# Tzq2doc/distributed_learning_simulator

Measured on AMD Instinct MI355X. Metric: FL rounds/sec (FedAvg, 100 clients, ResNet-18, CIFAR-10-shaped), higher is better.
Workload: dtype fp32; 1 GPU; fedavg_resnet18; model=ResNet18, algo=fed_avg, clients=100, local_epochs=5, global_batch=6400, per_client_batch=64, parallelism=client-dp1, backend=hip

## Files before the change

### csrc/bindings.cpp

```cpp
#include <pybind11/pybind11.h>

#include <algorithm>
#include <optional>
#include <stdexcept>
#include <string>
#include <vector>

#include "dls.h"

namespace py = pybind11;
typedef uintptr_t ptr;

template <typename T>
static T* P(ptr p) {
  return reinterpret_cast<T*>(p);
}
static hipStream_t S(ptr s) { return reinterpret_cast<hipStream_t>(s); }

extern "C" const char* dls_src_hash();

class Args {
 public:
  struct Ptr {
    uintptr_t v;
// ... 255 lines not shown
    p.coef = a.p("coef", 0); p.relu = a.i("relu", 0); p.x_valid = a.p("x_valid", 0);
    p.valid_img = a.p("valid_img", 0); p.dw = a.p("dw"); p.dw_cs = a.l("dw_cs"); p.part = a.p("part", 0);
    p.K = a.i("K"); p.B = a.i("B"); p.H = a.i("H"); p.W = a.i("W"); p.C = a.i("C"); p.N = a.i("N");
    const int xm = a.i("xm"), dm = a.i("dm");
    const hipStream_t s = a.p("s");
    a.finish();
    return halo_wgrad(p, xm, dm, s);
  });
  m.def("conv_halo_bn_dense_supported", &conv_halo_bn_dense_supported);
  m.def("conv_halo_bn_dense_fwd", [](py::kwargs kw) {
    Args a(kw, "conv_halo_bn_dense_fwd");
    const auto x = a.p("x"), coef = a.p("coef"), valid_rows = a.p("valid_rows", 0), wsplit = a.p("wsplit");
    const auto y = a.p("y"), stats = a.p("stats", 0), stats_valid = a.p("stats_valid", 0), s = a.p("s");
    const auto ny = a.p("ny", 0), mask = a.p("mask", 0);
    const long x_cs = a.l("x_cs"), ws_cs = a.l("ws_cs"), ws_plane = a.l("ws_plane"), y_cs = a.l("y_cs");
    const long ny_cs = a.l("ny_cs", 0);
    const int ldx = a.i("ldx"), creal = a.i("creal"), relu = a.i("relu", 0), rep = a.i("rep"), ldy = a.i("ldy");
    const int K = a.i("K"), B = a.i("B"), H = a.i("H"), W = a.i("W"), C = a.i("C"), N = a.i("N"), ldny = a.i("ldny", 0);
    a.finish();
    return conv_halo_bn_dense_fwd(x, x_cs, ldx, creal, coef, relu, valid_rows, wsplit, ws_cs, ws_plane, rep, y, y_cs,
                                  ldy, K, B, H, W, C, N, stats, stats_valid, ny, ny_cs, ldny, mask, s);
  });
  m.def("bn_bwd", [](py::kwargs kw) {
    Args a(kw, "bn_bwd");
    const auto dy = a.p("dy"), x = a.p("x"), y = a.p("y", 0), mean = a.p("mean", 0);
    const auto rstd = a.p("rstd", 0), gamma = a.p("gamma", 0), valid_rows = a.p("valid_rows", 0);
    const auto dx = a.p("dx", 0), dpre = a.p("dpre", 0), dgamma = a.p("dgamma", 0);
    const auto dbeta = a.p("dbeta", 0), ws = a.p("ws"), relu_mask = a.p("relu_mask", 0), s = a.p("s");
    const auto dxp = a.p("dxp", 0), pre_part = a.p("pre_part", 0), coef_ext = a.p("coef_ext", 0);
    const long g_cs = a.l("g_cs", 0), dg_cs = a.l("dg_cs", 0);
    const int K = a.i("K"), R = a.i("R"), C = a.i("C"), relu = a.i("relu", 0), f32 = a.i("f32");
    const int ldx = a.i("ldx", 0), acc_dx = a.i("acc_dx", 0), dx_f32 = a.i("dx_f32", 1);
    const int pre_nparts = a.i("pre_nparts", 0), stage = a.i("stage", 0);
    a.finish();
    bn_bwd(dy, x, y, mean, rstd, gamma, valid_rows, g_cs, K, R, C, relu, dx, dpre, dgamma, dbeta, dg_cs, ws, relu_mask,
           f32, s, ldx, acc_dx, dxp, dx_f32, pre_part, pre_nparts, coef_ext, stage);
  });
  m.def("ln_fwd", [](ptr x, ptr gamma, ptr beta, ptr y, ptr mean, ptr rstd, long g_cs, int K, long rpc, int C,
                     float eps, int rep, int f32, ptr s, ptr yp) {
    ln_fwd(P<const void>(x), P<const void>(gamma), P<const void>(beta), P<void>(y), P<float>(mean), P<float>(rstd),
           g_cs, K, rpc, C, eps, rep, f32, S(s), P<bf16_t>(yp));
  });
  m.def("ln_bwd", [](ptr dy, ptr x, ptr mean, ptr rstd, ptr gamma, long g_cs, int K, long rpc, int C, ptr dx,
                     ptr dgamma, ptr dbeta, long dg_cs, int f32, ptr s, ptr ws) {
    ln_bwd(P<const void>(dy), P<const void>(x), P<const float>(mean), P<const float>(rstd), P<const void>(gamma), g_cs,
           K, rpc, C, P<void>(dx), P<float>(dgamma), P<float>(dbeta), dg_cs, P<float>(ws), f32, S(s));
  });
  m.def("ln_workspace_floats", &ln_workspace_floats);
  m.def("gn_shape_ok", &gn_shape_ok);
  m.def("gn_workspace_floats", &gn_workspace_floats);
  m.def("gn_fwd", [](ptr x, ptr res, ptr gamma, ptr beta, ptr y, ptr yp, ptr mean, ptr rstd, ptr valid, long g_cs,
                     int rep, int K, int B, int HW, int C, int G, float eps, int relu, int f32, ptr s) {
    gn_fwd(P<const void>(x), P<const void>(res), P<const void>(gamma), P<const void>(beta), P<void>(y), P<bf16_t>(yp),
           P<float>(mean), P<float>(rstd), P<const int>(valid), g_cs, rep, K, B, HW, C, G, eps, relu, f32, S(s));
  });
  m.def("gn_bwd", [](ptr dy, ptr x, ptr y, ptr mean, ptr rstd, ptr gamma, ptr valid, long g_cs, int rep, int K, int B,
                     int HW, int C, int G, int relu, ptr dx, ptr dres, ptr dgamma, ptr dbeta, long dg_cs, ptr ws,
                     int f32, ptr s) {
    gn_bwd(P<const void>(dy), P<const void>(x), P<const void>(y), P<const float>(mean), P<const float>(rstd),
           P<const void>(gamma), P<const int>(valid), g_cs, rep, K, B, HW, C, G, relu, P<void>(dx), P<void>(dres),
           P<float>(dgamma), P<float>(dbeta), dg_cs, P<float>(ws), f32, S(s));
  });
  m.def("col_sum_workspace_floats", &col_sum_workspace_floats);
  m.def("col_sum", [](ptr x, ptr out, long out_cs, int K, long rows, int C, int f32, ptr s, ptr ws) {
    col_sum(P<const void>(x), P<float>(out), out_cs, K, rows, C, f32, S(s), P<float>(ws));
  });

  m.def("pool_fwd", [](ptr x, ptr y, ptr idx, int K, int B, int H, int W, int C, int OH, int OW, int k, int stride,
                       int pad, int mode, int f32, ptr s) {
// ... 248 lines not shown
```

### csrc/dls.h

```cpp
#pragma once
#include <hip/hip_runtime.h>
#include <stdint.h>

typedef uint16_t bf16_t;

constexpr int kOptUnset = -1000000;
extern int g_opt_attn_mfma, g_opt_conv_gl, g_opt_pl_min_wg;
extern int g_opt_halo_wgrad_unroll;
extern int g_opt_halo_skip;
extern int g_opt_conv_pix;
int native_option(int& slot, const char* env, int dflt);
bool set_native_option(const char* name, int value);

struct FastDiv {
  uint32_t d, mul, shift;
};

static inline FastDiv make_fastdiv(uint32_t d) {
  FastDiv f;
  f.d = d;
  uint32_t s = 0;
  while ((1u << s) < d) ++s;
  f.shift = s;
  f.mul = (uint32_t)((((uint64_t)1 << 32) * (((uint64_t)1 << s) - d)) / d + 1);
// ... 255 lines not shown
                 int ldy_x = 0, const int* valid_rows = nullptr);
void conv_halo_set_mode(int m);
void conv_halo_set_variant(int v);
bool conv_tn_pl_supported(const ConvTNParams& p);
bool conv_tn_pl(ConvTNParams p, int K, int variant, hipStream_t s);
int conv_tn_pl_num_variants();
int conv_tn_pl_variant();
void conv_tn_pl_set_variant(int v);
int conv_tn_pl_splitk(int K, int Co, int R, int M, int variant);
void tn_fold(const float* part, float* dw, long dw_cs, int K, int splitk, long CoR, hipStream_t s,
             const SgdEpi* sgd = nullptr);
int conv_tn_f32_num_variants();
int conv_tn_f32_splitk(int K, int Co, int R, int M, int gco, int gc, int variant);
bool conv_tn_f32_bn_bwd_ok(int K, int Co, int R, int gco, int gc, int variant);

long bn_workspace_floats(int K, long R, int C);
void bn_fwd(const void* x, const void* gamma, const void* beta, const void* res, void* y, float* mean, float* rstd,
            const int* valid_rows, long g_cs, int K, int R, int C, int relu, float eps, int rep, float* ws,
            uint8_t* relu_mask, int f32, hipStream_t s,
            int ldx = 0, const float* pre_part = nullptr,
            int pre_nparts = 0, bf16_t* yp = nullptr,
            int y_f32 = 1, float* coef_out = nullptr, int apply = 1,
            const float* res_coef = nullptr,
            int res_relu = 0);
void bn_bwd(const void* dy, const void* x, const void* y, const float* mean, const float* rstd, const void* gamma,
            const int* valid_rows, long g_cs, int K, int R, int C, int relu, void* dx, void* dpre, float* dgamma,
            float* dbeta, long dg_cs, float* ws, const uint8_t* relu_mask, int f32,
            hipStream_t s, int ldx = 0,
            int acc_dx = 0, bf16_t* dxp = nullptr,
            int dx_f32 = 1,
            const float* pre_part = nullptr,
            int pre_nparts = 0,
            float* coef_ext = nullptr,
            int stage = 0);
void ln_fwd(const void* x, const void* gamma, const void* beta, void* y, float* mean, float* rstd, long g_cs, int K,
            long rows_per_client, int C, float eps, int rep, int f32, hipStream_t s,
            bf16_t* yp = nullptr);
void ln_bwd(const void* dy, const void* x, const float* mean, const float* rstd, const void* gamma, long g_cs, int K,
            long rows_per_client, int C, void* dx, float* dgamma, float* dbeta, long dg_cs, float* ws, int f32,
            hipStream_t s);
long col_sum_workspace_floats(int K, long rows, int C);
long ln_workspace_floats(int K, long rows_per_client, int C);
bool gn_shape_ok(int HW, int C, int G);
long gn_workspace_floats(int K, int B, int C);
void gn_fwd(const void* x, const void* res, const void* gamma, const void* beta, void* y, bf16_t* yp, float* mean,
            float* rstd, const int* valid, long g_cs, int rep, int K, int B, int HW, int C, int G, float eps, int relu,
            int f32, hipStream_t s);
void gn_bwd(const void* dy, const void* x, const void* y, const float* mean, const float* rstd, const void* gamma,
            const int* valid, long g_cs, int rep, int K, int B, int HW, int C, int G, int relu, void* dx, void* dres,
            float* dgamma, float* dbeta, long dg_cs, float* ws, int f32, hipStream_t s);
void col_sum(const void* x, float* out, long out_cs, int K, long rows, int C, int f32, hipStream_t s,
             float* ws = nullptr);

void pool_fwd(const void* x, void* y, int* idx, int K, int B, int H, int W, int C, int OH, int OW, int k, int stride,
              int pad, int mode, int f32, hipStream_t s);
void pool_bwd(const void* dy, const int* idx, void* dx, int K, int B, int H, int W, int C, int OH, int OW, int k,
              int stride, int pad, int mode, int f32, hipStream_t s);
void gap_fwd(const void* x, void* y, int KB, int HW, int C, int f32, hipStream_t s);
void gap_bwd(const void* dy, void* dx, int KB, int HW, int C, int f32, hipStream_t s);
void ce_fwd_bwd(const void* logits, const int* labels, const int* valid, float* loss, float* correct, void* dlogits,
                int K, int B, int NC, int f32, hipStream_t s, float* rowbuf = nullptr);
void relu_bwd(const void* dy, const void* y, void* dx, long n, int f32, hipStream_t s);

void quant_pack(const float* x, long ld, const int* seg, const int64_t* seg_off, const int64_t* seg_numel,
                const uint8_t* bits, const float* lo, const float* scale, const int64_t* seg_byte_off,
                const int64_t* row_off, int K, int nseg, long P, int stochastic, const uint32_t* seeds, uint8_t* out,
                hipStream_t s);
// ... 140 lines not shown
```

### csrc/norm.hip

```cpp
#include "common.h"
#include <algorithm>
#include <numeric>

#include "dls.h"

namespace {

constexpr int ROWS_PER_BLOCK = 512;

static int rows_per_block(long R, int K) {
  const long want = std::min<long>(64, (2048 + K - 1) / K);
  const long bpc = std::max(1L, std::min(want, std::max(1L, R / 64)));
  return (int)std::min<long>(ROWS_PER_BLOCK, (R + bpc - 1) / bpc);
}

struct BNCoefArgs {
  const void* gamma;
  const void* beta;
  const float* mean_in;
  const float* rstd_in;
  float* mean_out;
  float* rstd_out;
  float* coef;
  float* dgamma;
  float* dbeta;
  long dg_cs, g_cs;
  float eps;
  int rep, bwd;
};

template <typename T>
__device__ __forceinline__ void bn_coef_math(float s0, float s1, int k, int c, int C, float n, const BNCoefArgs& a) {
  const long i = (long)k * C + c;
  const float g = ldf(static_cast<const T*>(a.gamma) + (long)(k / a.rep) * a.g_cs + c);
  if (!a.bwd) {
// ... 349 lines not shown
#pragma unroll
            for (int j = 0; j < V; ++j) out[j] += fmaxf(fmaf(rv[j], rsc[j], rsh[j]), 0.f);
          } else if (res_coef) {
#pragma unroll
            for (int j = 0; j < V; ++j) out[j] += fmaf(rv[j], rsc[j], rsh[j]);
          } else {
#pragma unroll
            for (int j = 0; j < V; ++j) out[j] += rv[j];
          }
        }
        if (relu) {
#pragma unroll
          for (int j = 0; j < V; ++j) out[j] = fmaxf(out[j], 0.f);
        }
      } else {
#pragma unroll
        for (int j = 0; j < V; ++j) out[j] = 0.f;
      }
      if (rmask) {
        uint32_t m = 0;
#pragma unroll
        for (int j = 0; j < V; ++j) m |= (rt<T>(out[j]) > 0.f ? 1u : 0u) << j;
        rmask[((long)k * R + r) * (C / 8) + c0 / 8] = (uint8_t)m;
      }
      if (y_f32) store_vec<V>(y + off, out);
      if (yp) {
        bf16_t* hp = yp + (long)k * R * C + off;
        store_planes<V>(hp, hp + (long)R * C, out);
      }
    }
  }
}

template <typename T, int V>
__global__ void __launch_bounds__(256) bn_bwd_apply_kernel(const T* __restrict__ dy, const T* __restrict__ x,
                                                           const T* __restrict__ y,
                                                           const int* __restrict__ valid_rows,
                                                           const float* __restrict__ coef, int R, int C, int relu,
                                                           T* __restrict__ dx, T* __restrict__ dpre,
                                                           int rpb, const uint8_t* __restrict__ rmask, int ldx,
                                                           int acc_dx, bf16_t* __restrict__ dxp, int dx_f32) {
  const int k = blockIdx.y;
  const int CT = C / V;
  const int nvalid = valid_rows ? min(valid_rows[k], R) : R;
  const int r0 = blockIdx.x * rpb, r1 = min(R, r0 + rpb);
  const long base = (long)k * R * C, base_x = (long)k * R * ldx;
  for (int cg = 0; cg < CT; cg += 256) {
    const int ctn = min(256, CT - cg);
    const int RT = 256 / ctn;
    const int cc = threadIdx.x % ctn, rl = threadIdx.x / ctn;
    if (rl >= RT) continue;
    const int c0 = (cg + cc) * V;
    float ca[V], cd[V], ce[V];
#pragma unroll
    for (int j = 0; j < V; ++j) {
      const long q = 3 * ((long)k * C + c0 + j);
      ca[j] = coef[q];
      cd[j] = coef[q + 1];
      ce[j] = coef[q + 2];
    }
    for (int r = r0 + rl; r < r1; r += RT) {
      const long off = base + (long)r * C + c0;
      const long offx = base_x + (long)r * ldx + c0;
      float o[V], gp[V];
      if (r < nvalid) {
        float vdy[V], vx[V];
        load_vec<V>(dy + off, vdy);
        load_vec<V>(x + offx, vx);
        if (rmask) {
          const uint32_t mbits = rmask[((long)k * R + r) * (C / 8) + c0 / 8];
#pragma unroll
          for (int j = 0; j < V; ++j) vdy[j] = ((mbits >> j) & 1u) ? vdy[j] : 0.f;
        } else if (relu) {
          float vy[V];
          load_vec<V>(y + off, vy);
#pragma unroll
          for (int j = 0; j < V; ++j) vdy[j] = vy[j] > 0.f ? vdy[j] : 0.f;
        }
#pragma unroll
        for (int j = 0; j < V; ++j) {
          gp[j] = vdy[j];
          o[j] = fmaf(ca[j], vdy[j], fmaf(ce[j], vx[j], cd[j]));
        }
      } else {
#pragma unroll
        for (int j = 0; j < V; ++j) o[j] = gp[j] = 0.f;
      }
      if (acc_dx) {
        float prev[V];
        load_vec<V>(dx + offx, prev);
#pragma unroll
        for (int j = 0; j < V; ++j) o[j] += prev[j];
// ... 256 lines not shown
                              (const float*)nullptr, (const float*)nullptr, mean, rstd, coef, (float*)nullptr,
                              (float*)nullptr, 0L, g_cs, K, R, C, eps, rep, 0, 0, 0L);
    } else {
      launch_coef<TT, float>(dim3(cdiv(C, 32), K), s, part, nparts, CP(gamma), CP(beta), valid_rows,
                             (const float*)nullptr, (const float*)nullptr, mean, rstd, coef, (float*)nullptr,
                             (float*)nullptr, 0L, g_cs, K, R, C, eps, rep, 0, 0, 0L);
    }
    if (apply) {
      DISPATCH_V(V, hipLaunchKernelGGL((bn_apply_kernel<TT, VV>), grid, dim3(256), 0, s, CP(x), CP(res), MP(y),
                                       valid_rows, coef, R, C, relu, rpb, rmask, ldx, f32 ? yp : nullptr,
                                       f32 ? y_f32 : 1, res_coef, res_relu));
    }
  });
}

void bn_apply_only(const float* x, const float* coef, const int* valid_rows, int K, int R, int C, int relu,
                   bf16_t* yp, uint8_t* rmask, hipStream_t s, float* y) {
  const int rpb = rows_per_block(R, K);
  dim3 grid(cdiv(R, rpb), K);
  if (C % 8 == 0) {
    hipLaunchKernelGGL((bn_apply_kernel<float, 8>), grid, dim3(256), 0, s, x, (const float*)nullptr, y,
                       valid_rows, coef, R, C, relu, rpb, rmask, C, yp, y ? 1 : 0, (const float*)nullptr, 0);
  } else {
    hipLaunchKernelGGL((bn_apply_kernel<float, 1>), grid, dim3(256), 0, s, x, (const float*)nullptr, y,
                       valid_rows, coef, R, C, relu, rpb, (uint8_t*)nullptr, C, yp, y ? 1 : 0, (const float*)nullptr,
                       0);
  }
}

void bn_bwd(const void* dy, const void* x, const void* y, const float* mean, const float* rstd, const void* gamma,
            const int* valid_rows, long g_cs, int K, int R, int C, int relu, void* dx, void* dpre, float* dgamma,
            float* dbeta, long dg_cs, float* ws, const uint8_t* rmask, int f32, hipStream_t s,
            int ldx, int acc_dx, bf16_t* dxp, int dx_f32, const float* pre_part, int pre_nparts, float* coef_ext,
            int stage) {
  if (!f32 || acc_dx || (ldx != 0 && ldx != C)) {
    dxp = nullptr;
    dx_f32 = 1;
  }
  if (ldx == 0) ldx = C;
  float* coef = coef_ext ? coef_ext : ws;
  float* part = ws + (long)3 * C * K;
  const int rpb = rows_per_block(R, K);
  dim3 grid(cdiv(R, rpb), K);
  const int V = vw(std::gcd(C, ldx));
  if (V != 8) rmask = nullptr;
  BNCoefArgs ca{gamma, nullptr, mean, rstd, nullptr, nullptr, coef, dgamma, dbeta, dg_cs, g_cs, 0.f, 1, 1};
  DISPATCH_T(f32, {
    if (stage == 2) {
    } else if (pre_part) {
      if (pre_nparts > FOLD && pre_nparts <= cdiv(R, 32)) {
        const int nfold = cdiv(pre_nparts, FOLD);
        double* folds = reinterpret_cast<double*>(ws + bn_fold_offset(K, R, C));
        hipLaunchKernelGGL(part_fold_kernel, dim3(nfold, K), dim3(256), 0, s, pre_part, pre_nparts, 2 * C, folds,
                           nfold);
        launch_coef<TT, double>(dim3(cdiv(C, 32), K), s, (const double*)folds, nfold, CP(gamma), (const TT*)nullptr,
                                valid_rows, mean, rstd, (float*)nullptr, (float*)nullptr, coef, dgamma, dbeta, dg_cs,
                                g_cs, K, R, C, 0.f, 1, 1, 0, 0L);
      } else {
        launch_coef<TT, float>(dim3(cdiv(C, 32), K), s, pre_part, pre_nparts, CP(gamma), (const TT*)nullptr,
                               valid_rows, mean, rstd, (float*)nullptr, (float*)nullptr, coef, dgamma, dbeta, dg_cs,
                               g_cs, K, R, C, 0.f, 1, 1, 0, 0L);
      }
    } else {
      DISPATCH_V(V, hipLaunchKernelGGL((chan_reduce_kernel<TT, VV, 1>), grid, dim3(256), 0, s, CP(dy), CP(x), CP(y),
                                       mean, rstd, valid_rows, R, C, relu, part, (long)2 * C, rpb, rmask, ca, C, ldx));
    }
    if (!pre_part && stage != 2)
      launch_coef<TT, float>(dim3(cdiv(C, 32), K), s, (const float*)part, (int)grid.x, CP(gamma), (const TT*)nullptr,
                             valid_rows, mean, rstd, (float*)nullptr, (float*)nullptr, coef, dgamma, dbeta, dg_cs, g_cs, K,
                             R, C, 0.f, 1, 1, 0, 0L);
    if (stage != 1)
      DISPATCH_V(V, hipLaunchKernelGGL((bn_bwd_apply_kernel<TT, VV>), grid, dim3(256), 0, s, CP(dy), CP(x), CP(y),
                                       valid_rows, coef, R, C, relu, MP(dx), MP(dpre), rpb, rmask, ldx, acc_dx, dxp,
                                       dx_f32));
  });
}

void fold_col_partials(const float* part, int nparts, int C, float* out, long out_cs, int K, hipStream_t s) {
  hipLaunchKernelGGL(part_sum_kernel, dim3(cdiv(C, 256), K), dim3(256), 0, s, part, nparts, C, C, out, (float*)nullptr,
                     out_cs);
}

void bn_bwd_coef_parts(const float* part, int nparts, const float* gamma, long g_cs, const int* valid_rows,
                       const float* mean, const float* rstd, int K, int R, int C, float* coef, float* dgamma,
                       float* dbeta, long dg_cs, hipStream_t s) {
  launch_coef<float, float>(dim3(cdiv(C, 32), K), s, part, nparts, gamma, (const float*)nullptr, valid_rows, mean, rstd,
                            (float*)nullptr, (float*)nullptr, coef, dgamma, dbeta, dg_cs, g_cs, K, R, C, 0.f, 1, 1, 0,
                            0L);
}

void part_sum_f64(const float* part, int K, int nparts, int g, double* out, long out_cs, int ldo, hipStream_t s) {
  if (K == 0) return;
  hipLaunchKernelGGL(part_sum_f64_kernel<float>, dim3(K), dim3(1024), 0, s, part, nparts, g, out, out_cs, ldo);
}

long chan_sums_f64_ws(int R, int C) { return (long)cdiv(R, 256) * 2 * C; }

void chan_sums_f64(const float* x, long x_cs, int ldx, int K, int R, int C, const int* valid, double* ws, double* out,
                   long out_cs, int ldo, hipStream_t s) {
  if (K == 0 || R == 0) return;
  const int rb = 256, nch = cdiv(R, rb);
  hipLaunchKernelGGL(chan_sums_f64_kernel, dim3(nch, K), dim3(256), 0, s, x, x_cs, ldx, R, C, valid, rb, ws, nch);
  hipLaunchKernelGGL(part_sum_f64_kernel<double>, dim3(K), dim3(1024), 0, s, (const double*)ws, nch, C, out, out_cs,
                     ldo);
}

void bn_coef_sums(const double* sums, long sums_cs, int ldp, const float* gamma, const float* beta,
// ... 76 lines not shown
```

### distributed_learning_simulator_amd/ops/functional.py

```python

from __future__ import annotations

import collections

import torch

from ..options import OPTIONS
from . import backend, ref
from .fusion import (BNBwdLink, BNOut, BNStats, DeferredBN, DeferredBNBwd, DeferredRes, DeferredStemBN,
                     MaskedGrad, ResidualLink, Tags, _require_fp32, bn_bwd_defer_count,
                     bn_bwd_f32_defer_count, bn_bwd_parts_count, res_fold_count, stem_defer_count, tag, tags)


def _be(t):
    return backend.get(t)


def _given(**kw):
    return {k: v for k, v in kw.items() if v is not None}


def _halo_shape(w, stride, pad) -> bool:
    return stride == 1 and pad == 1 and w.shape[2] == 3 and w.shape[3] == 3


def _stats_part(be, K, rows, C, device):
    return torch.empty((K, be.conv_stats_parts(rows), 2, C), dtype=torch.float32, device=device)


class _Conv(torch.autograd.Function):

    @staticmethod
    def forward(ctx, x, token, w, gw, stride, pad, b, gb, link=None, stats=None, w_split=None, donor=None,
                sgd=None):
        be = _be(x)
        ci = w.shape[-1]
        ctx.sgd = sgd if (sgd is not None and be is not ref and x.dtype == torch.float32 and gw is not None
                          and b is None and x.shape[-1] == ci and w_split is not None) else None
        if x.shape[-1] > ci:
            w = torch.nn.functional.pad(w, (0, x.shape[-1] - ci))
            w_split = None
        if be is ref or x.dtype != torch.float32:
            w_split = None
        tx = tags(x)
# ... 367 lines not shown
                be.linear_wgrad(dyc, x.unsqueeze(0).contiguous(), dw, None)
            ctx.gw.copy_(dw.view(K, Fo, Fi))
        return None, None, None, None


def linear_shared_input(x, token, w, gw):
    return _LinearSharedInput.apply(x, token, w, gw)


class _BN(torch.autograd.Function):
    @staticmethod
    def forward(ctx, x, token, gamma, beta, ggamma, gbeta, valid_rows, relu, residual, link=None, stats=None,
                planes=BNOut.FP32):
        be = _be(x)
        K = x.shape[0]
        C = x.shape[-1]
        _require_fp32(x, "batch_norm")
        x3 = x.reshape(K, -1, C)
        r3 = res_coef = None
        res_relu = False
        sdef = tags(residual).bn_defer
        if isinstance(sdef, DeferredStemBN):
            if (be is not ref and x.dtype == torch.float32 and sdef.y32 is None and sdef.valid_rows is valid_rows
                    and sdef.x.shape == x3.shape and x3.is_contiguous() and sdef.x.is_contiguous()):
                r3, res_coef, res_relu = sdef.x, sdef.coef, sdef.relu
                stem_defer_count["res"] += 1
            else:
                r3 = sdef.materialize_f32().reshape(K, -1, C)
        elif residual is not None:
            _require_fp32(residual, "batch_norm residual")
            r3 = residual.reshape(K, -1, C)
        mask = yp = bnb = defer = fold_out = None
        fold = tags(residual).res_fold
        if fold is not None and fold.pending:
            if (be is not ref and x.dtype == torch.float32 and fold.valid_rows is valid_rows
                    and fold.x.shape == x3.shape and x3.is_contiguous()):
                r3, res_coef = fold.x, fold.coef
                fold.taken("folded")
            else:
                fold.materialize()
        if be is ref:
            y, mean, rstd = be.bn_fwd(x3, gamma, beta, valid_rows, relu, r3)
        else:
            pre = stats.part if stats is not None else None
            planes = BNOut(planes) if (OPTIONS.planes and x.dtype == torch.float32 and x.is_contiguous()
                                       and be.planes_fit(x[0].numel())) else BNOut.FP32
            wm = any(ctx.needs_input_grad)
            C8 = C % 8 == 0
            can = {BNOut.CONV_DEFER: OPTIONS.bn_fused_halo and C8, BNOut.RES_FOLD: OPTIONS.bn_res_fold and not relu,
                   BNOut.STEM_DEFER: OPTIONS.bn_stem_defer and C8}
            if planes in can and not (can[planes] and residual is None and x3.is_contiguous()):
                planes = planes.applied_now
            if planes is BNOut.RES_FOLD:
                coef, mean, rstd = be.bn_coef(x3, gamma, beta, valid_rows, pre_stats=pre)
                y = torch.empty((K, x3.shape[1], C), dtype=x.dtype, device=x.device)
                fold_out = DeferredRes(x3, coef, valid_rows, y)
            elif planes in (BNOut.CONV_DEFER, BNOut.STEM_DEFER):
                coef, mean, rstd = be.bn_coef(x3, gamma, beta, valid_rows, pre_stats=pre)
                y, yp = be.planes_buffer((K, x3.shape[1], C), x.device)
                mask = torch.empty((K, x3.shape[1], C // 8), dtype=torch.uint8, device=x.device) if (wm and relu) else None
                defer = (DeferredBN if planes is BNOut.CONV_DEFER else DeferredStemBN)(x3, coef, relu, valid_rows, yp,
                                                                                       mask, write_out=wm)
            else:
                out = be.bn_fwd(x3, gamma, beta, valid_rows, relu, r3, with_mask=wm, pre_stats=pre, planes=int(planes),
                                res_coef=res_coef, res_relu=res_relu)
                y, mean, rstd = out[:3]
                mask = out[3] if wm else None
                if planes is not BNOut.FP32:
                    yp = out[-1]
            if stats is not None:
                stats.part = None
            if (wm and OPTIONS.bn_bwd_parts and x.dtype == torch.float32 and x3.is_contiguous()
                    and (mask is not None or not relu)):
                vr = valid_rows.to(torch.int32).contiguous() if valid_rows is not None else None
                bnb = BNBwdLink(x3, mask, mean, rstd, vr)
        ctx.save_for_backward(x3, y if mask is None else None, mean, rstd, gamma)
        ctx.relu_mask = mask
        ctx.valid_rows, ctx.relu, ctx.has_res = valid_rows, relu, residual is not None
        ctx.link = link
        ctx.stats = stats
        ctx.ggamma, ctx.gbeta, ctx.shape = ggamma, gbeta, x.shape
        ctx.bnb = bnb
        ctx.planes_on = OPTIONS.planes
        ctx.bwd_in_wgrad = OPTIONS.bn_bwd_in_wgrad
        ctx.bwd_in_wgrad_f32 = OPTIONS.bn_bwd_in_wgrad_f32
        yo = y.reshape(x.shape)
        if yp is not None:
            tag(yo, planes=yp.view((K, 2) + tuple(x.shape[1:])), planes_only=planes is not BNOut.BOTH)
        ctx.defer = defer
        if defer is not None or fold_out is not None or bnb is not None:
            tag(yo, bn_defer=defer, res_fold=fold_out, bnb=bnb)
        return yo

    @staticmethod
    def backward(ctx, dy):
        x3, y, mean, rstd, gamma = ctx.saved_tensors
        be = _be(dy)
        K, R, C = x3.shape
        if ctx.defer is not None:
            ctx.defer.materialize()
            ctx.defer = None
        dy3 = dy.reshape(K, R, C).contiguous()
        if be is ref:
            dx, dgamma, dbeta, dpre = ref.bn_bwd(dy3, x3, y, mean, rstd, gamma, ctx.valid_rows, ctx.relu)
            if ctx.ggamma is not None:
                ctx.ggamma.copy_(dgamma)
                ctx.gbeta.copy_(dbeta)
        else:
            _require_fp32(dy, "batch_norm backward")
            dxm = 2 if (ctx.stats is not None and ctx.stats.dy_planes_ok and ctx.planes_on) else 0
            pre = None
            bnb = ctx.bnb
            if bnb is not None:
                if bnb.part is not None and bnb.key == (dy3.data_ptr(), dy3._version):
                    pre = bnb.part
                bn_bwd_parts_count["used" if pre is not None else "none" if bnb.part is None else "fallback"] += 1
                bnb.part = bnb.key = None
            masked = (ctx.has_res and ctx.link is not None and ctx.relu and ctx.relu_mask is not None
                      and C % 8 == 0)
            if (dxm == 2 and ctx.bwd_in_wgrad and not (ctx.has_res and not masked) and C % 64 == 0
                    and (ctx.relu_mask is not None or not ctx.relu) and x3.is_contiguous()):
                coef = torch.empty((K, C, 3), dtype=torch.float32, device=dy3.device)
                be.bn_bwd(dy3, x3, y, mean, rstd, gamma, ctx.valid_rows, ctx.relu, ctx.ggamma, ctx.gbeta, False,
                          relu_mask=ctx.relu_mask, pre_part=pre, coef_out=coef)
                dx, dxp = be.planes_buffer((K, R, C), dy3.device)
                if masked:
                    ctx.link.grad = MaskedGrad(dy3.view(ctx.shape), ctx.relu_mask)
                dxo = dx.reshape(ctx.shape)
                tag(dxo, planes=dxp.view((K, 2) + tuple(ctx.shape[1:])), planes_only=True, bn_bwd=DeferredBNBwd(
                    dy3, x3, ctx.relu_mask if ctx.relu else None, coef, ctx.valid_rows, dxp))
                return dxo, None, None, None, None, None, None, None, None, None, None, None
            if (dxm == 0 and ctx.bwd_in_wgrad_f32 and ctx.stats is not None and ctx.stats.wgrad_bn_bwd_ok
                    and not ctx.has_res and C % 8 == 0 and (ctx.relu_mask is not None or not ctx.relu)
                    and x3.is_contiguous() and dy3.dtype == torch.float32):
                coef = torch.empty((K, C, 3), dtype=torch.float32, device=dy3.device)
                be.bn_bwd(dy3, x3, y, mean, rstd, gamma, ctx.valid_rows, ctx.relu, ctx.ggamma, ctx.gbeta, False,
                          relu_mask=ctx.relu_mask, pre_part=pre, coef_out=coef)
                dx = torch.empty((K, R, C), dtype=torch.float32, device=dy3.device)
                dxo = dx.reshape(ctx.shape)
                tag(dxo, planes_only=True, bn_bwd=DeferredBNBwd(
                    dy3, x3, ctx.relu_mask if ctx.relu else None, coef, ctx.valid_rows, dx, f32=True))
                return dxo, None, None, None, None, None, None, None, None, None, None, None
            out = be.bn_bwd(dy3, x3, y, mean, rstd, gamma, ctx.valid_rows, ctx.relu,
                            ctx.ggamma, ctx.gbeta, ctx.has_res and not masked, relu_mask=ctx.relu_mask,
                            dx_planes=dxm, pre_part=pre)
            dx, dpre = out[0], out[1]
            if masked:
                ctx.link.grad = MaskedGrad(dy3.view(ctx.shape), ctx.relu_mask)
            if dxm:
                dxo = dx.reshape(ctx.shape)
                tag(dxo, planes=out[2].view((K, 2) + tuple(ctx.shape[1:])), planes_only=True)
                dres = dpre.reshape(ctx.shape) if (ctx.has_res and not masked) else None
# ... 429 lines not shown
```

### distributed_learning_simulator_amd/ops/fusion.py

```python

from __future__ import annotations

import dataclasses
import enum

import torch


class BNOut(enum.IntEnum):

    FP32 = 0
    BOTH = 1
    PLANES = 2
    CONV_DEFER = 3
    RES_FOLD = 4
    STEM_DEFER = 5

    @property
    def applied_now(self) -> "BNOut":
        now = {BNOut.CONV_DEFER: BNOut.PLANES, BNOut.RES_FOLD: BNOut.FP32, BNOut.STEM_DEFER: BNOut.BOTH}
        return now.get(self, self)

    @property
    def reads_planes(self) -> bool:
# ... 122 lines not shown
        self.x, self.coef, self.relu, self.valid_rows = x, coef, relu, valid_rows
        self.yp, self.mask, self.write_out = yp, mask, write_out

    def _apply(self):
        from . import hip
        hip.bn_apply_only(self.x, self.coef, self.valid_rows, self.relu, self.yp, self.mask)


stem_defer_count = {"conv": 0, "res": 0, "materialized": 0}


class DeferredStemBN(DeferredBN):

    __slots__ = ("y32",)

    def __init__(self, x, coef, relu, valid_rows, yp, mask, write_out):
        super().__init__(x, coef, relu, valid_rows, yp, mask, write_out, stem_defer_count)
        self.y32 = None

    def materialize_f32(self):
        if self.y32 is None:
            from . import hip
            self.y32 = torch.empty(self.x.shape, dtype=self.x.dtype, device=self.x.device)
            hip.bn_apply_only(self.x, self.coef, self.valid_rows, self.relu, None, y=self.y32)
            self.count["materialized"] += 1
        return self.y32


res_fold_count = {"folded": 0, "materialized": 0}


class DeferredRes(Deferral):

    __slots__ = ("x", "coef", "valid_rows", "y")

    def __init__(self, x, coef, valid_rows, y):
        super().__init__(res_fold_count)
        self.x, self.coef, self.valid_rows, self.y = x, coef, valid_rows, y

    def _apply(self):
        from . import hip
        hip.bn_apply_only(self.x, self.coef, self.valid_rows, False, None, y=self.y)


bn_bwd_defer_count = {"wgrad": 0, "materialized": 0}
bn_bwd_f32_defer_count = {"wgrad": 0, "materialized": 0}


class DeferredBNBwd(Deferral):

    __slots__ = ("dy", "x", "mask", "coef", "valid_rows", "out", "f32")

    def __init__(self, dy, x, mask, coef, valid_rows, out, f32=False):
        super().__init__(bn_bwd_f32_defer_count if f32 else bn_bwd_defer_count)
        self.dy, self.x, self.mask, self.coef, self.valid_rows = dy, x, mask, coef, valid_rows
        self.out, self.f32 = out, f32

    def _apply(self):
        from . import hip
        apply = hip.bn_bwd_apply_f32 if self.f32 else hip.bn_bwd_apply_planes
        apply(self.dy, self.x, self.mask, self.coef, self.valid_rows, self.out)

    def wgrad_args(self):
        args = (self.dy, self.x, self.mask, self.coef, self.valid_rows)
        return args if self.f32 else args + (self.out,)
```

### distributed_learning_simulator_amd/ops/hip.py

```python

from __future__ import annotations

import collections
import importlib
import os
import threading

import torch

from ..options import OPTIONS
from . import ref

try:
    _C = importlib.import_module("distributed_learning_simulator_amd._dls_hip")
except ImportError as e:
    raise ImportError(
        "HIP extension _dls_hip is not built; run `python -m distributed_learning_simulator_amd.ops.build` "
        f"(original error: {e})"
    ) from e


def _check_provenance() -> None:
    from . import build as _build

# ... 854 lines not shown
    if dx_planes and dx_out is None and x.dtype == F32:
        dx, dxp = _planes_out((K, R, C), x.device, dx_planes)
    else:
        dx_planes = 0
        if dx_out is None:
            dx = torch.empty((K, R, C), dtype=x.dtype, device=x.device)
    dpre = torch.empty((K, R, C), dtype=x.dtype, device=x.device) if need_dpre else None
    ws = _workspace(_C.bn_workspace_floats(K, R, C), x.device)
    dg_cs = ggamma.stride(0) if ggamma is not None else 0
    assert dy.dtype == x.dtype == gamma.dtype
    if pre_part is not None:
        assert pre_part.dtype == F32 and pre_part.is_contiguous() and pre_part.shape == (K, (R + 31) // 32, 2, C)
    if coef_out is not None:
        assert coef_out.shape == (K, C, 3) and coef_out.dtype == F32 and coef_out.is_contiguous()
        assert dx_out is None and not need_dpre
    _C.bn_bwd(dy=_p(dy), x=_p(x), y=_p(y), mean=_p(mean), rstd=_p(rstd), gamma=_p(gamma), valid_rows=_pi32(valid_rows),
              g_cs=g_cs, K=K, R=R, C=C, relu=int(relu), dx=_p(dx), dpre=_p(dpre), dgamma=_p(ggamma), dbeta=_p(gbeta),
              dg_cs=dg_cs, ws=_p(ws), relu_mask=_p(relu_mask), f32=_f32(x), s=_s(), ldx=ldx, dxp=_p(dxp),
              acc_dx=int(dx_out is not None), dx_f32=int(dx_planes != 2), coef_ext=_p(coef_out),
              stage=1 if coef_out is not None else 0, **_pre_part(pre_part, K, C))
    if coef_out is not None:
        return None
    if dx_planes:
        return dx, dpre, dxp
    return dx, dpre


def bn_bwd_apply_planes(dy, x, relu_mask, coef, valid_rows, dxp) -> None:
    K, R, C = x.shape
    assert dxp.shape == (K, 2, R, C) and dxp.is_contiguous()
    _bn_bwd_apply(dy, x, relu_mask, coef, valid_rows, dx=_p(dxp), dxp=_p(dxp), dx_f32=0)


def bn_bwd_apply_f32(dy, x, relu_mask, coef, valid_rows, dx) -> None:
    assert dx.shape == x.shape and dx.dtype == F32 and dx.is_contiguous()
    _bn_bwd_apply(dy, x, relu_mask, coef, valid_rows, dx=_p(dx))


def _bn_bwd_apply(dy, x, relu_mask, coef, valid_rows, **out) -> None:
    K, R, C = x.shape
    assert dy.shape == x.shape and dy.is_contiguous() and x.is_contiguous() and dy.dtype == F32 == x.dtype
    assert coef.shape == (K, C, 3)
    ws = _workspace(_C.bn_workspace_floats(K, R, C), x.device)
    _C.bn_bwd(dy=_p(dy), x=_p(x), valid_rows=_pi32(valid_rows), K=K, R=R, C=C, relu=int(relu_mask is not None),
              ws=_p(ws), relu_mask=_p(relu_mask), f32=1, s=_s(), ldx=C, coef_ext=_p(coef), stage=2, **out)


def ln_fwd(x, gamma, beta, eps=1e-5, planes: bool = False):
    K = x.shape[0]
    C = x.shape[-1]
    x = x.contiguous()
    g_cs, rep = _client_view(gamma, K)
    rpc = x.numel() // (K * C)
    y = torch.empty_like(x)
    mean = torch.empty(x.shape[:-1], dtype=torch.float32, device=x.device)
    rstd = torch.empty_like(mean)
    assert gamma.dtype == x.dtype
    yp = torch.empty((K, 2) + tuple(x.shape[1:]), dtype=BF16, device=x.device) if planes and x.dtype == F32 else None
    _C.ln_fwd(_p(x), _p(gamma), _p(beta), _p(y), _p(mean), _p(rstd), g_cs, K, rpc, C, eps, rep, _f32(x), _s(), _p(yp))
    if planes:
        return y, mean, rstd, yp
    return y, mean, rstd


def ln_bwd(dy, x, mean, rstd, gamma):
    K = x.shape[0]
# ... 844 lines not shown
```

### distributed_learning_simulator_amd/options.py

```python

from __future__ import annotations

import contextlib
import dataclasses
import os
import threading


def _env_bool(name: str, default: bool) -> bool:
    v = os.environ.get(name)
    return default if v is None else v not in ("0", "", "false", "False")


def _env_int(name: str, default: int) -> int:
    v = os.environ.get(name)
    return default if v is None or v == "" else int(v)


@dataclasses.dataclass
class RuntimeOptions:
    planes: bool = dataclasses.field(default_factory=lambda: _env_bool("DLS_PLANES", True))
    """BatchNorms emit bf16 (hi, lo) planes for the LDS-DMA plane / halo GEMMs (off: every conv
    splits its operand in registers)."""
    fused_sgd: bool = dataclasses.field(default_factory=lambda: _env_bool("DLS_FUSED_SGD", True))
    """SGD steps of the weights whose plane / halo wgrad kernels can apply them (csrc/sgd_epi.h)
    run in those kernels; the flat step covers the rest (engine.params.FusedSGD)."""
    tfm_planes: bool = dataclasses.field(default_factory=lambda: _env_bool("DLS_TFM_PLANES", True))
    """Transformer split-plane producers: the FFN hidden activation and its gradient (linear1 /
    linear2 epilogues) and the dropout backward of the residual-branch linears (out_proj /
    linear2) write planes for the plane GEMMs (off: fp32 only). (Attention outputs writing planes
    measured +0.4-0.5 s per FedOBD stage-1 round each, profiles/r5_c6_ab_tfm_planes.txt: removed.)"""
    bn_bwd_parts: bool = dataclasses.field(default_factory=lambda: _env_bool("DLS_BN_BWD_PARTS", True))
    """BN backward partial sums from the consuming conv's dgrad epilogue (off: own reduction)."""
    bn_fused_halo: bool = dataclasses.field(default_factory=lambda: _env_bool("DLS_BN_FUSED_HALO", True))
    """A BN(+ReLU) whose only reader is a 3x3 stride-1 conv (ResNet BasicBlock bn1) is applied in
    that conv's halo loader (ops.fusion DeferredBN; off: BN apply pass + plane conv)."""
    bn_res_fold: bool = dataclasses.field(default_factory=lambda: _env_bool("DLS_BN_RES_FOLD", True))
    """A ResNet downsample shortcut's BN is applied inside the block's last BN apply, which reads
    its raw input as the residual (ops.fusion DeferredRes; off: its own apply pass)."""
    bn_stem_defer: bool = dataclasses.field(default_factory=lambda: _env_bool("DLS_BN_STEM_DEFER", True))
    """The CIFAR ResNet stem BN(+ReLU), read by layer1.0.conv1 (planes) and by layer1.0.bn2 (fp32, as
    its identity residual), is applied by those two readers: the conv in its halo loader, the BN
    in its residual fold (ops.fusion DeferredStemBN; off: one apply pass writes both forms)."""
    dense_bn_halo: bool = dataclasses.field(default_factory=lambda: _env_bool("DLS_DENSE_BN_HALO", True))
    """DenseNet growth convs apply their BN + ReLU in the halo loader over the block buffer's
    channel prefix (off: BN apply pass + implicit-GEMM conv)."""
    halo_wgrad: bool = dataclasses.field(default_factory=lambda: _env_bool("DLS_HALO_WGRAD", True))
    """3x3 stride-1 weight gradients of 64-512-channel convs (ResNet layers 1-3) on the LDS-halo
    kernel (csrc/conv_halo_wgrad.hip; off: the implicit-GEMM TN kernel)."""
    bn_bwd_in_wgrad: bool = dataclasses.field(default_factory=lambda: _env_bool("DLS_BN_BWD_IN_WGRAD", True))
    """A training BN(+ReLU) whose input gradient feeds only a 3x3 stride-1 conv's backward (ResNet
    BasicBlock bn1 / identity-block bn2, layers 1-3) computes its coefficients only: that conv's halo
    weight gradient applies the BN backward in its dY loader and writes dX's planes for the dgrad
    (ops.fusion DeferredBNBwd; off: the BN backward's own apply pass writes them)."""
    bn_bwd_in_wgrad_f32: bool = dataclasses.field(default_factory=lambda: _env_bool("DLS_BN_BWD_IN_WGRAD_F32", True))
    """A training BN(+ReLU) behind a conv whose input needs no gradient (the ResNet stem) computes
    its backward coefficients only: the conv's fp32 weight gradient applies the BN backward in its dY
    loader (ops.fusion DeferredBNBwd f32, csrc/conv_f32.hip; off: the BN backward's own apply pass
    writes dX and the weight gradient reads it back)."""
    dense_wgrad_halo: bool = dataclasses.field(default_factory=lambda: _env_bool("DLS_DENSE_WGRAD_HALO", True))
    """DenseNet growth-conv weight gradients on the LDS-halo kernel (the normalised prefix staged
    once per pixel tile for all nine taps; off: the implicit-GEMM TN kernel)."""
    dense_dgrad_fused: bool = dataclasses.field(default_factory=lambda: _env_bool("DLS_DENSE_DGRAD_FUSED", True))
    """DenseNet growth-conv input gradients fused with the BN backward (csrc/conv_dense_dgrad.hip:
    dX̂ recomputed in a sums pass and an apply pass instead of stored and read twice; off: the
    implicit-GEMM dgrad + the BN backward passes)."""
    dense_y_recompute: bool = dataclasses.field(default_factory=lambda: _env_bool("DLS_DENSE_Y_RECOMPUTE", True))
    """With the fused dgrad and the halo weight gradient, DenseNet training stores no normalised
    activation: both backward kernels rebuild relu(BN(x)) from the raw prefix and the forward's
    (scale, shift), bitwise (off: the forward's halo conv writes it for them)."""
    dense_stats_cache: bool = dataclasses.field(default_factory=lambda: _env_bool("DLS_DENSE_STATS_CACHE", True))
    """DenseNet blocks (fused growth convs) sum each channel's statistics once, from the producing
# ... 124 lines not shown
```

Measured before the change: 0.3001 rounds/s.

## Fold downsample shortcut BN backward into block's last BN backward apply

In a ResNet downsample block, the last BN's backward now also runs the shortcut BN's backward. Both reductions use the ReLU-mask-gated gradient, and one dual apply kernel writes both BNs' dX bf16 planes. The shortcut BN's backward then returns the parked planes instead of reading a dense fp32 gated gradient twice. This removes a materialized gradient tensor and a separate apply pass, at the cost of more Python-side plumbing and extra coefficient buffers.

```diff
diff --git a/csrc/bindings.cpp b/csrc/bindings.cpp
--- a/csrc/bindings.cpp
+++ b/csrc/bindings.cpp
@@ -311,9 +311,10 @@
     const int K = a.i("K"), R = a.i("R"), C = a.i("C"), relu = a.i("relu", 0), f32 = a.i("f32");
     const int ldx = a.i("ldx", 0), acc_dx = a.i("acc_dx", 0), dx_f32 = a.i("dx_f32", 1);
     const int pre_nparts = a.i("pre_nparts", 0), stage = a.i("stage", 0);
+    const auto x2 = a.p("x2", 0), coef2 = a.p("coef2", 0), dxp2 = a.p("dxp2", 0);
     a.finish();
     bn_bwd(dy, x, y, mean, rstd, gamma, valid_rows, g_cs, K, R, C, relu, dx, dpre, dgamma, dbeta, dg_cs, ws, relu_mask,
-           f32, s, ldx, acc_dx, dxp, dx_f32, pre_part, pre_nparts, coef_ext, stage);
+           f32, s, ldx, acc_dx, dxp, dx_f32, pre_part, pre_nparts, coef_ext, stage, x2, coef2, dxp2);
   });
   m.def("ln_fwd", [](ptr x, ptr gamma, ptr beta, ptr y, ptr mean, ptr rstd, long g_cs, int K, long rpc, int C,
                      float eps, int rep, int f32, ptr s, ptr yp) {
diff --git a/csrc/dls.h b/csrc/dls.h
--- a/csrc/dls.h
+++ b/csrc/dls.h
@@ -311,7 +311,10 @@
             const float* pre_part = nullptr,
             int pre_nparts = 0,
             float* coef_ext = nullptr,
-            int stage = 0);
+            int stage = 0,
+            const void* x2 = nullptr,
+            const float* coef2 = nullptr,
+            bf16_t* dxp2 = nullptr);
 void ln_fwd(const void* x, const void* gamma, const void* beta, void* y, float* mean, float* rstd, long g_cs, int K,
             long rows_per_client, int C, float eps, int rep, int f32, hipStream_t s,
             bf16_t* yp = nullptr);
diff --git a/csrc/norm.hip b/csrc/norm.hip
--- a/csrc/norm.hip
+++ b/csrc/norm.hip
@@ -1,6 +1,7 @@
 #include "common.h"
 #include <algorithm>
 #include <numeric>
+#include <stdexcept>
 
 #include "dls.h"
 
@@ -416,14 +417,16 @@
   }
 }
 
-template <typename T, int V>
+template <typename T, int V, int DUAL = 0>
 __global__ void __launch_bounds__(256) bn_bwd_apply_kernel(const T* __restrict__ dy, const T* __restrict__ x,
                                                            const T* __restrict__ y,
                                                            const int* __restrict__ valid_rows,
                                                            const float* __restrict__ coef, int R, int C, int relu,
                                                            T* __restrict__ dx, T* __restrict__ dpre,
                                                            int rpb, const uint8_t* __restrict__ rmask, int ldx,
-                                                           int acc_dx, bf16_t* __restrict__ dxp, int dx_f32) {
+                                                           int acc_dx, bf16_t* __restrict__ dxp, int dx_f32,
+                                                           const T* __restrict__ x2, const float* __restrict__ coef2,
+                                                           bf16_t* __restrict__ dxp2) {
   const int k = blockIdx.y;
   const int CT = C / V;
   const int nvalid = valid_rows ? min(valid_rows[k], R) : R;
@@ -442,6 +445,42 @@
       ca[j] = coef[q];
       cd[j] = coef[q + 1];
       ce[j] = coef[q + 2];
+    }
+    if constexpr (DUAL) {
+      float ca2[V], cd2[V], ce2[V];
+#pragma unroll
+      for (int j = 0; j < V; ++j) {
+        const long q = 3 * ((long)k * C + c0 + j);
+        ca2[j] = coef2[q];
+        cd2[j] = coef2[q + 1];
+        ce2[j] = coef2[q + 2];
+      }
+      for (int r = r0 + rl; r < r1; r += RT) {
+        const long off = base + (long)r * C + c0;
+        float o[V], o2[V];
+        if (r < nvalid) {
+          float vdy[V], vx[V], vx2[V];
+          load_vec<V>(dy + off, vdy);
+          load_vec<V>(x + off, vx);
+          load_vec<V>(x2 + off, vx2);
+          const uint32_t mbits = rmask[((long)k * R + r) * (C / 8) + c0 / 8];
+#pragma unroll
+          for (int j = 0; j < V; ++j) vdy[j] = ((mbits >> j) & 1u) ? vdy[j] : 0.f;
+#pragma unroll
+          for (int j = 0; j < V; ++j) {
+            o[j] = fmaf(ca[j], vdy[j], fmaf(ce[j], vx[j], cd[j]));
+            o2[j] = fmaf(ca2[j], vdy[j], fmaf(ce2[j], vx2[j], cd2[j]));
+          }
+        } else {
+#pragma unroll
+          for (int j = 0; j < V; ++j) o[j] = o2[j] = 0.f;
+        }
+        bf16_t* hp = dxp + (long)k * R * C + off;
+        store_planes<V>(hp, hp + (long)R * C, o);
+        bf16_t* hp2 = dxp2 + (long)k * R * C + off;
+        store_planes<V>(hp2, hp2 + (long)R * C, o2);
+      }
+      continue;
     }
     for (int r = r0 + rl; r < r1; r += RT) {
       const long off = base + (long)r * C + c0;
@@ -764,7 +803,19 @@
             const int* valid_rows, long g_cs, int K, int R, int C, int relu, void* dx, void* dpre, float* dgamma,
             float* dbeta, long dg_cs, float* ws, const uint8_t* rmask, int f32, hipStream_t s,
             int ldx, int acc_dx, bf16_t* dxp, int dx_f32, const float* pre_part, int pre_nparts, float* coef_ext,
-            int stage) {
+            int stage, const void* x2, const float* coef2, bf16_t* dxp2) {
+  if (x2 || coef2 || dxp2) {
+    if (!(x2 && coef2 && dxp2 && coef_ext && dxp && rmask && stage == 2 && f32 && C % 8 == 0 && !acc_dx && !dx_f32 &&
+          !dpre && (ldx == 0 || ldx == C)))
+      throw std::invalid_argument("bn_bwd: the two-BN apply takes fp32 contiguous operands with C % 8 == 0, a ReLU "
+                                  "mask, stage 2 and planes-only outputs");
+    const int rpb2 = rows_per_block(R, K);
+    hipLaunchKernelGGL((bn_bwd_apply_kernel<float, 8, 1>), dim3(cdiv(R, rpb2), K), dim3(256), 0, s,
+                       static_cast<const float*>(dy), static_cast<const float*>(x), (const float*)nullptr, valid_rows,
+                       (const float*)coef_ext, R, C, 1, (float*)nullptr, (float*)nullptr, rpb2, rmask, C, 0, dxp, 0,
+                       static_cast<const float*>(x2), coef2, dxp2);
+    return;
+  }
   if (!f32 || acc_dx || (ldx != 0 && ldx != C)) {
     dxp = nullptr;
     dx_f32 = 1;
@@ -804,7 +855,7 @@
     if (stage != 1)
       DISPATCH_V(V, hipLaunchKernelGGL((bn_bwd_apply_kernel<TT, VV>), grid, dim3(256), 0, s, CP(dy), CP(x), CP(y),
                                        valid_rows, coef, R, C, relu, MP(dx), MP(dpre), rpb, rmask, ldx, acc_dx, dxp,
-                                       dx_f32));
+                                       dx_f32, (const TT*)nullptr, (const float*)nullptr, (bf16_t*)nullptr));
   });
 }
 
diff --git a/distributed_learning_simulator_amd/ops/functional.py b/distributed_learning_simulator_amd/ops/functional.py
--- a/distributed_learning_simulator_amd/ops/functional.py
+++ b/distributed_learning_simulator_amd/ops/functional.py
@@ -9,7 +9,8 @@
 from . import backend, ref
 from .fusion import (BNBwdLink, BNOut, BNStats, DeferredBN, DeferredBNBwd, DeferredRes, DeferredStemBN,
                      MaskedGrad, ResidualLink, Tags, _require_fp32, bn_bwd_defer_count,
-                     bn_bwd_f32_defer_count, bn_bwd_parts_count, res_fold_count, stem_defer_count, tag, tags)
+                     bn_bwd_f32_defer_count, bn_bwd_parts_count, res_bwd_fold_count, res_fold_count, stem_defer_count,
+                     tag, tags)
 
 
 def _be(t):
@@ -443,11 +444,15 @@
             r3 = residual.reshape(K, -1, C)
         mask = yp = bnb = defer = fold_out = None
         fold = tags(residual).res_fold
+        ctx.res_fold = None
+        ctx.res_ds = fold is not None
         if fold is not None and fold.pending:
             if (be is not ref and x.dtype == torch.float32 and fold.valid_rows is valid_rows
                     and fold.x.shape == x3.shape and x3.is_contiguous()):
                 r3, res_coef = fold.x, fold.coef
                 fold.taken("folded")
+                if OPTIONS.bn_ds_bwd_fold and fold.bwd is not None and any(ctx.needs_input_grad):
+                    ctx.res_fold = fold
             else:
                 fold.materialize()
         if be is ref:
@@ -466,6 +471,9 @@
                 coef, mean, rstd = be.bn_coef(x3, gamma, beta, valid_rows, pre_stats=pre)
                 y = torch.empty((K, x3.shape[1], C), dtype=x.dtype, device=x.device)
                 fold_out = DeferredRes(x3, coef, valid_rows, y)
+                if wm:
+                    fold_out.set_bwd(mean, rstd, gamma, ggamma, gbeta,
+                                     stats is not None and stats.dy_planes_ok and OPTIONS.planes)
             elif planes in (BNOut.CONV_DEFER, BNOut.STEM_DEFER):
                 coef, mean, rstd = be.bn_coef(x3, gamma, beta, valid_rows, pre_stats=pre)
                 y, yp = be.planes_buffer((K, x3.shape[1], C), x.device)
@@ -499,6 +507,7 @@
         if yp is not None:
             tag(yo, planes=yp.view((K, 2) + tuple(x.shape[1:])), planes_only=planes is not BNOut.BOTH)
         ctx.defer = defer
+        ctx.res_out = fold_out
         if defer is not None or fold_out is not None or bnb is not None:
             tag(yo, bn_defer=defer, res_fold=fold_out, bnb=bnb)
         return yo
@@ -527,8 +536,35 @@
                     pre = bnb.part
                 bn_bwd_parts_count["used" if pre is not None else "none" if bnb.part is None else "fallback"] += 1
                 bnb.part = bnb.key = None
+            parked = ctx.res_out.dx if ctx.res_out is not None else None
+            if parked is not None:
+                ctx.res_out.dx = None
+                dxo = parked[0].reshape(ctx.shape)
+                tag(dxo, planes=parked[1].view((K, 2) + tuple(ctx.shape[1:])), planes_only=True)
+                return dxo, None, None, None, None, None, None, None, None, None, None, None
             masked = (ctx.has_res and ctx.link is not None and ctx.relu and ctx.relu_mask is not None
                       and C % 8 == 0)
+            fold = ctx.res_fold
+            if (fold is not None and dxm == 2 and fold.bwd[5] and not masked and ctx.relu
+                    and dy3.dtype == torch.float32 and fold.valid_rows is ctx.valid_rows
+                    and be.bn_bwd_apply_planes2_ok(x3, fold.x, ctx.relu_mask)):
+                ds_mean, ds_rstd, ds_gamma, ds_ggamma, ds_gbeta, _ = fold.bwd
+                coef = torch.empty((K, C, 3), dtype=torch.float32, device=dy3.device)
+                ds_coef = torch.empty((K, C, 3), dtype=torch.float32, device=dy3.device)
+                be.bn_bwd(dy3, x3, y, mean, rstd, gamma, ctx.valid_rows, True, ctx.ggamma, ctx.gbeta, False,
+                          relu_mask=ctx.relu_mask, pre_part=pre, coef_out=coef)
+                be.bn_bwd(dy3, fold.x, None, ds_mean, ds_rstd, ds_gamma, ctx.valid_rows, True, ds_ggamma, ds_gbeta,
+                          False, relu_mask=ctx.relu_mask, coef_out=ds_coef)
+                dx, dxp = be.planes_buffer((K, R, C), dy3.device)
+                fold.dx = be.planes_buffer((K, R, C), dy3.device)
+                be.bn_bwd_apply_planes2(dy3, ctx.relu_mask, (x3, coef, dxp), (fold.x, ds_coef, fold.dx[1]),
+                                        ctx.valid_rows)
+                res_bwd_fold_count["folded"] += 1
+                dxo = dx.reshape(ctx.shape)
+                tag(dxo, planes=dxp.view((K, 2) + tuple(ctx.shape[1:])), planes_only=True)
+                return dxo, None, None, None, None, None, None, None, dy, None, None, None
+            if ctx.res_ds:
+                res_bwd_fold_count["separate"] += 1
             if (dxm == 2 and ctx.bwd_in_wgrad and not (ctx.has_res and not masked) and C % 64 == 0
                     and (ctx.relu_mask is not None or not ctx.relu) and x3.is_contiguous()):
                 coef = torch.empty((K, C, 3), dtype=torch.float32, device=dy3.device)
diff --git a/distributed_learning_simulator_amd/ops/fusion.py b/distributed_learning_simulator_amd/ops/fusion.py
--- a/distributed_learning_simulator_amd/ops/fusion.py
+++ b/distributed_learning_simulator_amd/ops/fusion.py
@@ -178,15 +178,26 @@
 
 class DeferredRes(Deferral):
 
-    __slots__ = ("x", "coef", "valid_rows", "y")
+    __slots__ = ("x", "coef", "valid_rows", "y", "bwd", "dx")
 
     def __init__(self, x, coef, valid_rows, y):
         super().__init__(res_fold_count)
         self.x, self.coef, self.valid_rows, self.y = x, coef, valid_rows, y
+        self.bwd = self.dx = None
+
+    def set_bwd(self, mean, rstd, gamma, ggamma, gbeta, dx_planes_ok: bool):
+        self.bwd = (mean, rstd, gamma, ggamma, gbeta, dx_planes_ok)
+
+    def taken(self, key: str):
+        super().taken(key)
+        self.y = None
 
     def _apply(self):
         from . import hip
         hip.bn_apply_only(self.x, self.coef, self.valid_rows, False, None, y=self.y)
+
+
+res_bwd_fold_count = {"folded": 0, "separate": 0}
 
 
 bn_bwd_defer_count = {"wgrad": 0, "materialized": 0}
diff --git a/distributed_learning_simulator_amd/ops/hip.py b/distributed_learning_simulator_amd/ops/hip.py
--- a/distributed_learning_simulator_amd/ops/hip.py
+++ b/distributed_learning_simulator_amd/ops/hip.py
@@ -910,6 +910,27 @@
     _bn_bwd_apply(dy, x, relu_mask, coef, valid_rows, dx=_p(dxp), dxp=_p(dxp), dx_f32=0)
 
 
+def bn_bwd_apply_planes2_ok(x, x2, relu_mask) -> bool:
+    return (relu_mask is not None and x.dtype == F32 == x2.dtype and x.shape == x2.shape and x.shape[-1] % 8 == 0
+            and x.is_contiguous() and x2.is_contiguous())
+
+
+def bn_bwd_apply_planes2(dy, relu_mask, bn, bn2, valid_rows) -> None:
+    (x, coef, dxp), (x2, coef2, dxp2) = bn, bn2
+    K, R, C = x.shape
+    assert bn_bwd_apply_planes2_ok(x, x2, relu_mask), "bn_bwd_apply_planes2: fp32 contiguous [K, R, C % 8 == 0] + mask"
+    assert dy.shape == x.shape and dy.is_contiguous() and dy.dtype == F32
+    assert relu_mask.shape == (K, R, C // 8) and relu_mask.dtype == torch.uint8 and relu_mask.is_contiguous()
+    for cf, dp in ((coef, dxp), (coef2, dxp2)):
+        assert cf.shape == (K, C, 3) and cf.dtype == F32 and cf.is_contiguous()
+        assert dp.shape == (K, 2, R, C) and dp.dtype == torch.bfloat16 and dp.is_contiguous()
+    assert coef.data_ptr() != coef2.data_ptr() and dxp.data_ptr() != dxp2.data_ptr()
+    ws = _workspace(_C.bn_workspace_floats(K, R, C), x.device)
+    _C.bn_bwd(dy=_p(dy), x=_p(x), valid_rows=_pi32(valid_rows), K=K, R=R, C=C, relu=1, ws=_p(ws),
+              relu_mask=_p(relu_mask), f32=1, s=_s(), ldx=C, coef_ext=_p(coef), stage=2, dx=_p(dxp), dxp=_p(dxp),
+              dx_f32=0, x2=_p(x2), coef2=_p(coef2), dxp2=_p(dxp2))
+
+
 def bn_bwd_apply_f32(dy, x, relu_mask, coef, valid_rows, dx) -> None:
     assert dx.shape == x.shape and dx.dtype == F32 and dx.is_contiguous()
     _bn_bwd_apply(dy, x, relu_mask, coef, valid_rows, dx=_p(dx))
diff --git a/distributed_learning_simulator_amd/options.py b/distributed_learning_simulator_amd/options.py
--- a/distributed_learning_simulator_amd/options.py
+++ b/distributed_learning_simulator_amd/options.py
@@ -38,6 +38,11 @@
     bn_res_fold: bool = dataclasses.field(default_factory=lambda: _env_bool("DLS_BN_RES_FOLD", True))
     """A ResNet downsample shortcut's BN is applied inside the block's last BN apply, which reads
     its raw input as the residual (ops.fusion DeferredRes; off: its own apply pass)."""
+    bn_ds_bwd_fold: bool = dataclasses.field(default_factory=lambda: _env_bool("DLS_BN_DS_BWD_FOLD", True))
+    """The backward half of bn_res_fold: the block's last BN, whose backward gates dy by its ReLU
+    bits, also runs the shortcut BN's backward on that gated gradient — its reduction with the same
+    bits, then one apply pass that writes both BNs' dX planes (ops.fusion DeferredRes; off: it writes
+    the gated gradient as a dense fp32 tensor and the shortcut BN's own backward reads it twice)."""
     bn_stem_defer: bool = dataclasses.field(default_factory=lambda: _env_bool("DLS_BN_STEM_DEFER", True))
     """The CIFAR ResNet stem BN(+ReLU), read by layer1.0.conv1 (planes) and by layer1.0.bn2 (fp32, as
     its identity residual), is applied by those two readers: the conv in its halo loader, the BN
```

After: 0.3030 rounds/s, median of 6. Within noise of the previous version (+1.0%).
